# kchmck/p25rx

Hardware: AMD Instinct MI355X
Metric: IQ Msamples/s through FM-demod+C4FM slice (higher is better)
Workload: dtype f32

## Files before the change

### p25rx_amd/csrc/p25fe_api.hip

```cpp
#include "p25fe_kernels.hip"

#include <hip/hip_ext.h>
#include <math.h>
#include <stdio.h>
#include <stdlib.h>
#include <string.h>

#include <chrono>
#include <new>
#include <utility>
#include <string>
#include <vector>

#include "p25fe_jit.h"

using namespace p25k;

namespace {

constexpr size_t BBPAD = 256;
constexpr size_t SHARD_HALO = 2560;
static_assert(SHARD_HALO >= (size_t)(DEC * (PLPAD + CLK_L + 160) + TMAX) && 160 >= TMAX + TMAX - 1 && SHARD_HALO % 8 == 0, "shard halo");
constexpr uint32_t STATE_MAGIC = 0x50323546u;

// ... 685 lines not shown
}
struct K1Launch {
    const void* src = nullptr;
    int fmt = P25FE_FMT_CF32;
    size_t ch_stride = 0, n_hist = 0, n = 0;
    uint64_t abs0 = 0;
    float* bb = nullptr; size_t bb_stride = 0;
    float* power_dbm = nullptr;
    bool planar = false;
    K1Part part = K1_ALL;
    hipEvent_t ev0 = nullptr, ev1 = nullptr;
    const ChunkRecvArgs* chunk = nullptr;
    long* head_end = nullptr;
    unsigned* done_flag = nullptr; unsigned done_seq = 0u;
    hipStream_t stream = nullptr;
};

struct K1Plan {
    bool empty;
    K1Args a;
    int fmt, variant; bool ct; int pk;
    long n_seg;
    long head_end;
    size_t lds;
};
static int k1_plan(const p25fe_t* h, const K1Launch& L, K1Plan* p)
{
    const int fmt = L.fmt;
    const int variant = format_variant_of(h->variant, h->dflt, h->cfg.specialize, fmt);
    if (variant < 0) return variant;
    if ((reinterpret_cast<uintptr_t>(L.src) & 15u) != 0) return P25FE_ERR_ARG;
    if (h->C > 1 && (L.ch_stride % fmt_stride_unit(fmt)) != 0) return P25FE_ERR_ARG;
    if (L.chunk && (!L.planar || L.part)) return P25FE_ERR_ARG;
    const bool pro = seg_prologue(fmt);
    const long m_begin = !L.planar ? 0 : (pro ? -(long)PLPAD - h->look : -(long)HIST_BB - h->look);
    const size_t n_out = p25fe_n_baseband_h(h, L.abs0, L.n);
    const long total = (long)n_out - m_begin;
    K1Args& a = p->a;
    a.m_begin = m_begin; a.n_out = (long)n_out; p->head_end = 0;
    p->empty = total <= 0;
    if (p->empty) return P25FE_OK;
    const int pk = (L.planar || h->long_taps || variant == P25FE_VARIANT_SPECIALIZED) ? 5 : h->k1_p;
    const int t1 = h->long_taps ? TMAX : T1;
    static const long subs_env = [] { const char* e = getenv("P25FE_SUBS"); return e ? atol(e) : 0L; }();
    long subs = subs_env > 0 ? subs_env : (fmt == P25FE_FMT_U8 ? 9 : (fmt == P25FE_FMT_S16 ? P25FE_K1_SUBS_S16 : 3));
    if (L.chunk) subs = 1;
    if (subs > 32768) subs = 32768;
    const bool ct = variant != P25FE_VARIANT_GENERIC;
    const int t2e = h->long_taps ? TMAX : T2;
    const int t3geo = ct ? h->n_avg : TMAX;
    SegGeo g{pro, WV * pk, (int)subs, seg_halo_for(h->n_avg, t2e), 0, m_begin, (long)n_out};
    const int nd = g.front(t3geo, t2e);
    const long o0 = (long)(((uint64_t)h->phase + 5 - L.abs0 % 5) % 5);
    if (L.part && subs > 1 && !L.chunk) g.set_lead(nd, o0, t1);
    const long n_seg = g.count(total);
    const long pl_shift = PLPAD + h->look;
    if (L.planar && !g.planar_ok(pl_shift)) return P25FE_ERR_ARG;
    if (L.planar && n_out > MAX_RANGE_BB) return P25FE_ERR_ARG;
    long seg_first = 0, seg_count = n_seg;
    if (L.part) {
        if (L.power_dbm) return P25FE_ERR_ARG;
        const long k_min = g.head_count(n_seg, nd, o0, t1);
        if (L.part == K1_MAIN) { seg_first = k_min; seg_count = n_seg - k_min; }
        else seg_count = k_min;
        p->head_end = g.start(k_min) - m_begin;
        p->empty = seg_count <= 0;
        if (p->empty) return P25FE_OK;
    }
    if (seg_count * (long)h->C > 0x7fffffffL) return P25FE_ERR_ARG;
    p->fmt = fmt; p->variant = variant; p->ct = ct; p->pk = pk; p->n_seg = n_seg;
    a.x = L.src; a.ch_stride = (long)L.ch_stride; a.n_hist = (long)L.n_hist; a.n_new = (long)L.n; a.o0 = (int)o0; a.n_ch = h->C;
    a.bb = L.bb; a.bb_stride = (long)L.bb_stride; a.power_partial = nullptr;
    a.subs_per_seg = g.subs_per_seg; a.seg_first = (int)seg_first; a.seg_count = (int)seg_count; a.lead_segs = g.lead_segs; a.seg_halo = g.segh;
    a.bbp = nullptr; a.bbp_ch_stride = 0; a.bits = nullptr; a.bits_ch_stride = 0; a.pl_shift = (int)pl_shift;
    a.done_flag = L.planar ? L.done_flag : nullptr; a.done_seq = L.done_seq;
    if (L.planar) {
        const PlanarGeo g(n_out);
        a.bbp = h->rx().pl_f.get(); a.bbp_ch_stride = (long)g.floats();
        a.bits = reinterpret_cast<uint8_t*>(h->rx().pl_bits.get()); a.bits_ch_stride = (long)(4 * g.words());
    }
    const bool lut = fmt == P25FE_FMT_U8 && (!ct || h->u8_lut_mode);
    p->lds = h->long_taps ? k1_lds_bytes<Geo<5, 1>>(ct, lut, t3geo) : (pk == 3 ? k1_lds_bytes<Geo<3>>(ct, lut, t3geo) : k1_lds_bytes<Geo<5>>(ct, lut, t3geo));
    static const size_t lds_pad_env = [] { const char* e = getenv("P25FE_K1_LDS_PAD"); return e ? (size_t)atol(e) : (size_t)0; }();
    p->lds += lds_pad_env;
    return P25FE_OK;
}

using K1Kernel = void (*)(K1Args, const Taps*);
using ChunkKernel = void (*)(K1Args, const Taps*, ChunkTail);
template <int FMT> static K1Kernel k1_kernel_of(bool ct, int pk, bool planar, bool long_taps)
{
    if (long_taps) return planar ? k_frontend<FMT, false, 5, OUT_PLANAR, 1> : k_frontend<FMT, false, 5, OUT_LINEAR, 1>;
    if (planar) return ct ? k_frontend<FMT, true, 5, OUT_PLANAR, 0> : k_frontend<FMT, false, 5, OUT_PLANAR, 0>;
    if (pk == 3) return ct ? k_frontend<FMT, true, 3, OUT_LINEAR, 0> : k_frontend<FMT, false, 3, OUT_LINEAR, 0>;
    return ct ? k_frontend<FMT, true, 5, OUT_LINEAR, 0> : k_frontend<FMT, false, 5, OUT_LINEAR, 0>;
}
template <int FMT> static ChunkKernel chunk_kernel_of(bool ct, bool long_taps)
{
    if (long_taps) return k_chunk<FMT, false, 1>;
    return ct ? k_chunk<FMT, true, 0> : k_chunk<FMT, false, 0>;
}
static K1Kernel k1_kernel_of(int fmt, bool ct, int pk, bool planar, bool long_taps)
{
    switch (fmt) {
    case P25FE_FMT_U8: return k1_kernel_of<P25FE_FMT_U8>(ct, pk, planar, long_taps);
    case P25FE_FMT_S16: return k1_kernel_of<P25FE_FMT_S16>(ct, pk, planar, long_taps);
    default: return k1_kernel_of<P25FE_FMT_CF32>(ct, pk, planar, long_taps);
    }
}
static ChunkKernel chunk_kernel_of(int fmt, bool ct, bool long_taps)
{
    switch (fmt) {
    case P25FE_FMT_U8: return chunk_kernel_of<P25FE_FMT_U8>(ct, long_taps);
    case P25FE_FMT_S16: return chunk_kernel_of<P25FE_FMT_S16>(ct, long_taps);
    default: return chunk_kernel_of<P25FE_FMT_CF32>(ct, long_taps);
// ... 1427 lines not shown
```

### p25rx_amd/csrc/p25fe_jit.cpp

```cpp
#include "p25fe_jit.h"

#include <dlfcn.h>
#include <errno.h>
#include <fcntl.h>
#include <hip/hiprtc.h>
#include <math.h>
#include <stdio.h>
#include <stdlib.h>
#include <string.h>
#include <sys/stat.h>
#include <sys/types.h>
#include <unistd.h>

#include "p25fe_embed.inc"

namespace p25jit {

const char* const KERNEL_NAMES[2][3] = {
    {"p25jit_k1_cf32_lin", "p25jit_k1_cf32_pl", "p25jit_chunk_cf32"},
    {"p25jit_k1_u8_lin", "p25jit_k1_u8_pl", "p25jit_chunk_u8"},
};

static const char* const OPTIONS[] = {"--offload-arch=gfx950", "-O3", "-std=c++17", "-ffp-contract=off", "-fno-fast-math",
                                      "-fhip-fp32-correctly-rounded-divide-sqrt", "-Wno-unused-function"};
static const int N_OPTIONS = (int)(sizeof OPTIONS / sizeof OPTIONS[0]);

static const char WRAPPER[] =
    "#include \"p25fe_jit_spec.h\"\n"
    "#include \"p25fe_kernels.hip\"\n"
    "using namespace p25k;\n"
    "#define P25JIT_K1(NAME, FMT, OM, WPS) extern \"C\" __global__ __launch_bounds__(WV, WPS) void NAME(K1Args a, const Taps* __restrict__ t) "
    "{ frontend_body<FMT, true, 5, OM, P25FE_JIT_TX>(a, t); }\n"
    "P25JIT_K1(p25jit_k1_cf32_lin, P25FE_FMT_CF32, OUT_LINEAR, Geo<5>::WAVES_PER_SIMD)\n"
    "P25JIT_K1(p25jit_k1_u8_lin, P25FE_FMT_U8, OUT_LINEAR, Geo<5>::WAVES_PER_SIMD)\n"
    "P25JIT_K1(p25jit_k1_cf32_pl, P25FE_FMT_CF32, OUT_PLANAR, P25FE_K1_PLANAR_WPS)\n"
    "P25JIT_K1(p25jit_k1_u8_pl, P25FE_FMT_U8, OUT_PLANAR, (P25FE_JIT_AVG_N > AVG_DPP_MAX ? 2 : P25FE_K1_PLANAR_WPS_U8))\n"
    "extern \"C\" __global__ __launch_bounds__(WV, 2) void p25jit_chunk_cf32(K1Args a, const Taps* __restrict__ t, ChunkTail c) "
    "{ chunk_body<P25FE_FMT_CF32, true, P25FE_JIT_TX>(a, t, c); }\n"
    "extern \"C\" __global__ __launch_bounds__(WV, 2) void p25jit_chunk_u8(K1Args a, const Taps* __restrict__ t, ChunkTail c) "
    "{ chunk_body<P25FE_FMT_U8, true, P25FE_JIT_TX>(a, t, c); }\n";

namespace rtc {
struct Api {
    void* lib = nullptr;
    decltype(&hiprtcCreateProgram) create = nullptr;
    decltype(&hiprtcCompileProgram) compile = nullptr;
    decltype(&hiprtcGetProgramLogSize) log_size = nullptr;
    decltype(&hiprtcGetProgramLog) log = nullptr;
    decltype(&hiprtcGetCodeSize) code_size = nullptr;
    decltype(&hiprtcGetCode) code = nullptr;
    decltype(&hiprtcDestroyProgram) destroy = nullptr;
    decltype(&hiprtcGetErrorString) error_string = nullptr;
    decltype(&hiprtcVersion) version = nullptr;
    bool ok = false;
};
static const Api& api()
{
    static const Api a = [] {
        Api x;
        const char* env = getenv("P25FE_HIPRTC");
        const char* names[] = {"libhiprtc.so.7", "libhiprtc.so", "/opt/rocm/lib/libhiprtc.so"};
        if (env && *env) x.lib = dlopen(env, RTLD_NOW | RTLD_LOCAL);
        else
            for (const char* n : names)
                if ((x.lib = dlopen(n, RTLD_NOW | RTLD_LOCAL)) != nullptr) break;
        if (!x.lib) return x;
#define P25_SYM(field, name) x.field = reinterpret_cast<decltype(x.field)>(dlsym(x.lib, name))
        P25_SYM(create, "hiprtcCreateProgram"); P25_SYM(compile, "hiprtcCompileProgram");
// ... 262 lines not shown
```

### p25rx_amd/csrc/p25fe_kernels.hip

```cpp
#ifndef __HIPCC_RTC__
#include <hip/hip_runtime.h>
#include <stdint.h>
#endif

#include "p25fe.h"
#include "p25fe_spec.h"

namespace p25k {

#ifdef P25FE_MEASURE
#include "p25fe_measure.inc"
#else
#define P25FE_M_LOAD_OFFSET(product_, cached_row_) (product_)
#define P25FE_M_ENTRY do { } while (0)
#define P25FE_M_LOCALS do { } while (0)
#define P25FE_M_ITEM do { } while (0)
#define P25FE_M_SUBTILE do { } while (0)
#define P25FE_M_EXIT do { } while (0)
#define K1_STAMP(i) do { } while (0)
#define K1_PIN2(a, b) do { } while (0)
#define P25FE_M_PIN_V2(arr_, n_) do { } while (0)
#define P25FE_M_PIN_F2(arr_, n_) do { } while (0)
#define P25FE_M_CUT_LOADS do { } while (0)
#define P25FE_M_CUT(stage_) do { } while (0)
// ... 21 lines not shown
#define K1_CT_DECIM_TAPS P25FE_JIT_DECIM_TAPS
#define K1_CT_CHAN_TAPS P25FE_JIT_CHAN_TAPS
#define K1_CT_FM_GAIN P25FE_JIT_FM_GAIN
#define K1_CT_U8_SCALE P25FE_JIT_U8_SCALE
#define K1_CT_U8_OFFSET P25FE_JIT_U8_OFFSET
#define K1_CT_U8_LUT P25FE_JIT_U8_LUT
#define K1_CT_AVG_N P25FE_JIT_AVG_N
#define K1_CT_AVG_TAPS P25FE_JIT_AVG_TAPS
#define K1_CT_AVG_UNIFORM P25FE_JIT_AVG_UNIFORM
#else
#define K1_CT_DECIM_TAPS P25FE_DEFAULT_DECIM_TAPS
#define K1_CT_CHAN_TAPS P25FE_DEFAULT_CHAN_TAPS
#define K1_CT_FM_GAIN P25FE_FM_GAIN
#define K1_CT_U8_SCALE P25FE_U8_SCALE
#define K1_CT_U8_OFFSET P25FE_U8_OFFSET
#define K1_CT_U8_LUT 0
#define K1_CT_AVG_N P25FE_BOXCAR
#define K1_CT_AVG_TAPS P25FE_DEFAULT_AVG_TAPS
#define K1_CT_AVG_UNIFORM 1
#endif

constexpr int WV = 64;
constexpr int DEC = P25FE_DECIM;
constexpr int T1 = P25FE_T1;
constexpr int T2 = P25FE_T2;
constexpr int BOX = P25FE_BOXCAR;
constexpr int HALO_Y = BOX;
constexpr int HALO_D = HALO_Y + (T2 - 1);
constexpr int TMAX = P25FE_MAX_TAPS;
constexpr int AVG_DPP_MAX = 11;
constexpr int SEG_HALO = 80;
__host__ __device__ constexpr int seg_halo_for(int t3, int t2) { return t3 + t2 - 1 <= 80 ? 80 : 160; }
static_assert(SEG_HALO == seg_halo_for(BOX, TMAX) && seg_halo_for(TMAX, TMAX) >= TMAX + TMAX - 1, "segment halo covers the filter memory and is byte-aligned per plane");
#ifndef P25FE_K1_PRO_CF32
#define P25FE_K1_PRO_CF32 0
#endif
#ifndef P25FE_K1_PRO_S16
#define P25FE_K1_PRO_S16 1
#endif
__host__ __device__ constexpr bool seg_prologue(int fmt)
{
    return fmt == P25FE_FMT_U8 ? true : (fmt == P25FE_FMT_S16 ? P25FE_K1_PRO_S16 != 0 : P25FE_K1_PRO_CF32 != 0);
}
__host__ __device__ constexpr int fmt_bps(int fmt) { return fmt == P25FE_FMT_CF32 ? 8 : (fmt == P25FE_FMT_S16 ? 4 : 2); }

constexpr int SPS_ = P25FE_SPS;
constexpr int PLPAD = 320;
static_assert(PLPAD % 320 == 0 && PLPAD >= 240 + 2, "planar pad holds the receiver's history");
constexpr int OUT_LINEAR = 0, OUT_PLANAR = 1;
constexpr int PL_BLK = 32 * P25FE_SPS;
__host__ __device__ inline long planar_index(long i, int r) { return (i >> 5) * PL_BLK + r * 32 + (i & 31); }

#define K1_GEO_FN __host__ __device__ __forceinline__ constexpr
#define K1_FIRST_INPUT(m, o0, t1) ((long)(o0) + DEC * (m) - ((t1) - 1))
struct SegGeo {
    bool pro;
    int sub, subs_per_seg;
    int segh;
    int lead_segs;
    long m_begin, n_out;
    long seg_len_ = pro ? (long)subs_per_seg * sub : (long)(sub - segh) + (long)(subs_per_seg - 1) * sub;
    long lead_len_ = pro ? (long)sub : (long)(sub - segh);
    K1_GEO_FN long seg_len() const { return seg_len_; }
    K1_GEO_FN long lead_len() const { return lead_len_; }
    K1_GEO_FN SegGeo range(int lead, long mb, long no) const { SegGeo g = *this; g.lead_segs = lead; g.m_begin = mb; g.n_out = no; return g; }
    K1_GEO_FN bool is_lead(long k) const { return k < (long)lead_segs; }
    K1_GEO_FN long len(long k) const { return is_lead(k) ? lead_len_ : seg_len_; }
    K1_GEO_FN int subs(long k) const { return is_lead(k) ? 1 : subs_per_seg; }
    K1_GEO_FN long start(long k) const { return m_begin + (is_lead(k) ? k * lead_len_ : (long)lead_segs * lead_len_ + (k - lead_segs) * seg_len_); }
    K1_GEO_FN long end_of(long m0, long len_) const { return (m0 + len_ < n_out) ? m0 + len_ : n_out; }
    K1_GEO_FN long end(long k) const { return end_of(start(k), len(k)); }
    K1_GEO_FN long count(long total) const
    {
        return lead_segs * lead_len_ >= total ? (total + lead_len_ - 1) / lead_len_ : lead_segs + (total - lead_segs * lead_len_ + seg_len_ - 1) / seg_len_;
    }
    K1_GEO_FN int front(int t3geo, int t2) const { return pro ? t3geo + t2 - 1 : segh; }
    K1_GEO_FN static long first_input(long m, long o0, int t1) { return K1_FIRST_INPUT(m, o0, t1); }
    K1_GEO_FN bool in_head(long k, int front_, long o0, int t1) const { return first_input(start(k) - front_, o0, t1) < 0; }
    K1_GEO_FN long head_count(long n_seg, int front_, long o0, int t1) const { long k = 0; while (k < n_seg && in_head(k, front_, o0, t1)) ++k; return k; }
    K1_GEO_FN void set_lead(int front_, long o0, int t1) { for (lead_segs = 0; lead_segs < 64 && start(lead_segs) < n_out && in_head(lead_segs, front_, o0, t1);) ++lead_segs; }
    K1_GEO_FN bool planar_ok(long pl_shift) const
    {
// ... 3 lines not shown
};
#undef K1_GEO_FN
constexpr int HIST_IQ = DEC * HALO_D + (T1 - 1) + (DEC - 1);
constexpr int HIST_IQ_MAX = DEC * (TMAX + TMAX - 1) + (TMAX - 1) + (DEC - 1);

template <int PK, int TX = 0> struct Geo {
    static constexpr int T1 = TX ? TMAX : P25FE_T1;
    static constexpr int T2 = TX ? TMAX : P25FE_T2;
    static constexpr int D_CARRY = (T2 - 1 + 1) & ~1;
    static constexpr int P = PK;
    static constexpr int SUB = WV * PK;
    static constexpr int XWIN = DEC * SUB + (T1 - DEC);
    static constexpr int XIN_N = (XWIN + 1 + 7) / 8 * 8;
    static constexpr int D_N = D_CARRY + SUB;
    static constexpr int TAPS_N = T1 + T2 + 3 + TMAX + 1;
    static constexpr size_t LDS_BASE = sizeof(float2) * (D_CARRY + XIN_N);
    static_assert(sizeof(float2) * XIN_N >= sizeof(float2) * SUB + sizeof(float) * SUB, "d and the transpose fit the window region");
    static constexpr int WAVES_PER_SIMD = PK <= 3 ? 4 : 2;
};

struct Taps {
    float dec[TMAX];
    float ch[TMAX];
    float lut[256];
    float fm_gain;
    int n_avg;
    int avg_uniform;
    float pad_;
    float avg[TMAX];
};
#ifndef P25FE_K1_AVG_LDS_CF32
#define P25FE_K1_AVG_LDS_CF32 0
#endif
template <class G> __host__ __device__ constexpr size_t k1_lds_bytes(bool ct, bool lut, int t3)
{
    return G::LDS_BASE + sizeof(float) * (size_t)((ct ? 0 : G::TAPS_N) + (lut ? 256 : 0) + (t3 > AVG_DPP_MAX || !ct || P25FE_K1_AVG_LDS_CF32 ? t3 - 1 + G::SUB : 0));
}

__device__ __forceinline__ float spec_atan2f(float y, float x)
{
    const float ax = __builtin_fabsf(x), ay = __builtin_fabsf(y);
    const float mx = ax > ay ? ax : ay;
    const float mn = ax > ay ? ay : ax;
    const float t = mn / mx;
    const float s = t * t;
    float p = P25FE_ATAN_COEFFS[P25FE_ATAN_NCOEF - 1];
#pragma unroll
    for (int i = P25FE_ATAN_NCOEF - 2; i >= 0; --i) p = __builtin_fmaf(p, s, P25FE_ATAN_COEFFS[i]);
    float r = p * t;
    if (ay > ax) r = P25FE_HALF_PI - r;
    if (x < 0.0f) r = P25FE_PI - r;
    if (y < 0.0f) r = -r;
    return mx == 0.0f ? 0.0f : r;
}

__device__ __forceinline__ float fm_discriminate(float2 s, float2 prev, float gain)
{
    const float t = s.y * prev.y;
    const float re = __builtin_fmaf(s.x, prev.x, t);
    const float u = s.x * prev.y;
    const float im = __builtin_fmaf(s.y, prev.x, -u);
    return spec_atan2f(im, re) * gain;
}

typedef float v2f __attribute__((ext_vector_type(2)));
#ifndef P25FE_K1_SCALAR_FMA
#define P25FE_K1_SCALAR_FMA 0
#endif
__device__ __forceinline__ v2f cfma(float tap, v2f s, v2f acc)
// ... 147 lines not shown
        "v_writelane_b32 %0, %1, 0\n\tv_writelane_b32 %0, %2, 5\n\t"
        "v_writelane_b32 %0, %3, 1\n\tv_writelane_b32 %0, %4, 6\n\t"
        "v_writelane_b32 %0, %5, 2\n\tv_writelane_b32 %0, %6, 7\n\t"
        "v_writelane_b32 %0, %7, 3\n\tv_writelane_b32 %0, %8, 8\n\t"
        "v_writelane_b32 %0, %9, 4\n\tv_writelane_b32 %0, %10, 9"
        : "+v"(v)
        : "s"((unsigned)m[0]), "s"((unsigned)(m[0] >> 32)), "s"((unsigned)m[1]), "s"((unsigned)(m[1] >> 32)),
          "s"((unsigned)m[2]), "s"((unsigned)(m[2] >> 32)), "s"((unsigned)m[3]), "s"((unsigned)(m[3] >> 32)),
          "s"((unsigned)m[4]), "s"((unsigned)(m[4] >> 32)));
    return v;
}
__device__ __forceinline__ unsigned lane_gather(unsigned v, int src)
{
    return (unsigned)__builtin_amdgcn_ds_bpermute(src << 2, (int)v);
}

__device__ __forceinline__ void phase_sync()
{
    __builtin_amdgcn_fence(__ATOMIC_RELEASE, "wavefront");
    __builtin_amdgcn_wave_barrier();
    __builtin_amdgcn_fence(__ATOMIC_ACQUIRE, "wavefront");
}

__device__ __forceinline__ float u8_to_f32(unsigned b) { return __builtin_fmaf((float)b, K1_CT_U8_SCALE, K1_CT_U8_OFFSET); }
__device__ __forceinline__ float2 s16_to_c32(unsigned w)
{
    const int i = (int)(short)(w & 0xffffu), q = (int)w >> 16;
    return make_float2((float)i * P25FE_S16_SCALE, (float)q * P25FE_S16_SCALE);
}

#ifndef P25FE_K1_LD_AUX
#define P25FE_K1_LD_AUX 0
#endif
template <int FMT, int PK, int TX = 0, int NVX = 0> struct Loader {
    using G = Geo<PK, TX>;
    static constexpr int LOG_SPV = 1;
    static constexpr int SPV = 1 << LOG_SPV;
    static constexpr int NV = NVX ? NVX : (G::XWIN + SPV + SPV * WV - 1) / (SPV * WV);
    static_assert(FMT == P25FE_FMT_CF32 || FMT == P25FE_FMT_S16 || FMT == P25FE_FMT_U8, "input format");
    using V = typename cond<FMT == P25FE_FMT_CF32, uint4, typename cond<FMT == P25FE_FMT_S16, uint2, unsigned>::type>::type;
    V v[NV];

    typedef unsigned v4u_t __attribute__((ext_vector_type(4)));
    typedef unsigned v2u_t __attribute__((ext_vector_type(2)));
    static constexpr int BPS = fmt_bps(FMT);
    static constexpr int VB = BPS * SPV;
    __device__ __forceinline__ void load_vec(int j, int o)
    {
        if constexpr (FMT == P25FE_FMT_CF32) {
            const v4u_t t = __builtin_amdgcn_raw_buffer_load_b128(rs, o, 0, P25FE_K1_LD_AUX);
            v[j] = make_uint4(t.x, t.y, t.z, t.w);
        } else if constexpr (FMT == P25FE_FMT_S16) {
            const v2u_t t = __builtin_amdgcn_raw_buffer_load_b64(rs, o, 0, P25FE_K1_LD_AUX);
            v[j] = make_uint2(t.x, t.y);
        } else {
            v[j] = __builtin_amdgcn_raw_buffer_load_b32(rs, o, 0, P25FE_K1_LD_AUX);
        }
    }
    __amdgpu_buffer_rsrc_t rs;
    long base_idx;

    __device__ __forceinline__ void init(const void* base, long first0, long n_hist, long n_new, long i_last)
    {
        const long f_al = (first0 >> LOG_SPV) << LOG_SPV;
        const long lo_al = ((-n_hist) >> LOG_SPV) << LOG_SPV;
        base_idx = f_al > lo_al ? f_al : lo_al;
        const long last = i_last < n_new - 1 ? i_last : n_new - 1;
        long bytes = ((last + 1 - base_idx + SPV - 1) >> LOG_SPV) * VB;
        bytes = bytes < 0 ? 0 : (bytes > (1L << 30) ? (1L << 30) : bytes);
        const uintptr_t p = reinterpret_cast<uintptr_t>(base) + (uintptr_t)(base_idx * BPS);
        const unsigned plo = __builtin_amdgcn_readfirstlane((unsigned)p), phi = __builtin_amdgcn_readfirstlane((unsigned)(p >> 32));
        rs = __builtin_amdgcn_make_buffer_rsrc(reinterpret_cast<void*>(((uintptr_t)phi << 32) | plo), 0,
                                               __builtin_amdgcn_readfirstlane((int)bytes), 0x00020000);
    }
    __device__ __forceinline__ void load_first(long first, int tid)
    {
        const long f_al = (first >> LOG_SPV) << LOG_SPV;
        long rel = (f_al - base_idx) * BPS;
        rel = rel < -(1L << 30) ? -(1L << 30) : (rel > (1L << 30) ? (1L << 30) : rel);
        const int voff = (int)rel + VB * tid;
#pragma unroll
        for (int j = 0; j < NV; ++j) {
            int o = voff + j * VB * WV;
            o = o < 0 ? 0x7ffffff0 : o;
            load_vec(j, o);
        }
    }
    __device__ __forceinline__ void load(long first, int tid)
    {
        const long f_al = (first >> LOG_SPV) << LOG_SPV;
        long rel = (f_al - base_idx) * BPS;
        rel = rel < -(1L << 30) ? -(1L << 30) : (rel > (1L << 30) ? (1L << 30) : rel);
        const int voff = (int)rel + VB * tid;
#pragma unroll
        for (int j = 0; j < NV; ++j) {
            const int o = P25FE_M_LOAD_OFFSET(voff + j * VB * WV, VB * tid);
            load_vec(j, o);
        }
    }

    template <bool LUTM = false>
    __device__ __forceinline__ void store(float2* XIN, long first, long n_hist, long n_new, int tid, const float* lut = nullptr) const
    {
        float4* XV = reinterpret_cast<float4*>(__builtin_assume_aligned(XIN, 16));
#pragma unroll
        for (int j = 0; j < NV; ++j) {
            float2 s[SPV];
#pragma unroll
            for (int e = 0; e < SPV; ++e) {
                if constexpr (FMT == P25FE_FMT_CF32) {
                    const unsigned w[4] = {v[j].x, v[j].y, v[j].z, v[j].w};
                    s[e] = make_float2(__uint_as_float(w[2 * e]), __uint_as_float(w[2 * e + 1]));
                } else if constexpr (FMT == P25FE_FMT_S16) {
                    s[e] = s16_to_c32(e ? v[j].y : v[j].x);
                } else {
                    const unsigned pair = (v[j] >> (16 * e)) & 0xffffu;
                    if constexpr (LUTM) s[e] = make_float2(lut[pair & 0xffu], lut[pair >> 8]);
                    else s[e] = make_float2(u8_to_f32(pair & 0xffu), u8_to_f32(pair >> 8));
                }
            }
            if (j < NV - 1 || SPV * (tid + j * WV) + SPV <= G::XIN_N) XV[tid + j * WV] = make_float4(s[0].x, s[0].y, s[1].x, s[1].y);
        }
    }
    __device__ __forceinline__ void fixup(float2* XIN, long first, long n_hist, long n_new, int tid) const
    {
        const long first_al = (first >> LOG_SPV) << LOG_SPV;
        if (first_al >= -n_hist && first_al + (long)NV * SPV * WV <= n_new) return;
#pragma unroll
        for (int j = 0; j < NV; ++j)
#pragma unroll
            for (int e = 0; e < SPV; ++e) {
                const long i = first_al + SPV * (long)(tid + j * WV) + e;
                const int k = SPV * (tid + j * WV) + e;
                if ((i < -n_hist || i >= n_new) && k < G::XIN_N) XIN[k] = make_float2(0.f, 0.f);
            }
    }
};

struct K1Args {
    const void* x;
    long ch_stride;
    long n_hist;
    long n_new;
    int o0;
    float* bb;
    long bb_stride;
    long n_out;
    int subs_per_seg;
    int seg_count;
    int n_ch;
    int seg_first;
    long m_begin;
    float* power_partial;
    float* bbp;
    long bbp_ch_stride;
    uint8_t* bits;
    long bits_ch_stride;
    int pl_shift;
    unsigned* done_flag;
    unsigned done_seq;
    int lead_segs;
    int seg_halo;
};

#ifndef P25FE_K1_PLANAR_WPS
#define P25FE_K1_PLANAR_WPS 2
#endif
#ifndef P25FE_K1_PLANAR_WPS_U8
#define P25FE_K1_PLANAR_WPS_U8 3
#endif
#ifndef P25FE_K1_PLANAR_WPS_S16
#define P25FE_K1_PLANAR_WPS_S16 3
#endif
#ifndef P25FE_K1_TURNAROUND_PRIO
#define P25FE_K1_TURNAROUND_PRIO 3
#endif
#ifndef P25FE_K1_PF_CF32
#define P25FE_K1_PF_CF32 1
#endif
#ifndef P25FE_K1_NT_STORES
#define P25FE_K1_NT_STORES 1
#endif
#ifndef P25FE_K1_PF_U8
#define P25FE_K1_PF_U8 2
#endif
#ifndef P25FE_K1_SUBS_S16
#define P25FE_K1_SUBS_S16 9
#endif
#ifndef P25FE_K1_PF_S16
#define P25FE_K1_PF_S16 1
#endif
template <int FMT, bool CT, int PK, int OM = OUT_LINEAR, int TX = 0>
__device__ __forceinline__ void frontend_body(const K1Args& a, const Taps* __restrict__ gtaps)
{
    constexpr int PF = (PK != 5 || TX != 0) ? 1 : (FMT == P25FE_FMT_U8 ? P25FE_K1_PF_U8 : (FMT == P25FE_FMT_S16 ? P25FE_K1_PF_S16 : P25FE_K1_PF_CF32));
#ifndef P25FE_JIT
    static_assert(TX == 0 || !CT, "the 64-tap geometry is for caller-supplied taps");
#endif
    static_assert(OM == OUT_LINEAR || PK == 5, "the planar epilogue maps a 320-sample sub-tile onto 10 planes x 32 symbols");
    P25FE_M_ENTRY;
    using G = Geo<PK, TX>;
    constexpr int SUB = G::SUB;
    constexpr int P = PK;
    constexpr int T1 = G::T1, T2 = G::T2, D_CARRY = G::D_CARRY;
    constexpr int T3 = CT ? K1_CT_AVG_N : TMAX;
    constexpr bool AVG_DPP = CT && T3 <= AVG_DPP_MAX && !(P25FE_K1_AVG_LDS_CF32 != 0 && FMT == P25FE_FMT_CF32);
    constexpr int HY = T3;
    constexpr int NBACK = AVG_DPP ? ((T3 - 1 + PK - 1) / PK > 0 ? (T3 - 1 + PK - 1) / PK : 1) : 1;
    static_assert(T3 >= 1 && T3 <= TMAX && NBACK <= 3, "post-discriminator filter length");
    extern __shared__ __attribute__((aligned(16))) char smem[];
    float2* D = reinterpret_cast<float2*>(smem);
    float2* XIN = D + D_CARRY;
    float* OUT = reinterpret_cast<float*>(D + G::D_N);
    float* TAPS = reinterpret_cast<float*>(D + D_CARRY + G::XIN_N);
    float* const LUT = TAPS + (CT ? 0 : G::TAPS_N);
    float* const AVT = TAPS + (T1 + T2 + 3);
    constexpr bool LUTM = FMT == P25FE_FMT_U8 && (!CT || K1_CT_U8_LUT != 0);
    const int tid = threadIdx.x;
    if (!CT) {
        for (int k = tid; k < T1; k += WV) TAPS[k] = gtaps->dec[k];
        for (int k = tid; k < T2; k += WV) TAPS[T1 + k] = gtaps->ch[k];
        for (int k = tid; k < TMAX; k += WV) AVT[k] = gtaps->avg[k];
    }
    if constexpr (LUTM)
        for (int k = tid; k < 256; k += WV) LUT[k] = gtaps->lut[k];
    float* const FM = LUT + (LUTM ? 256 : 0);
    float fm_gain = K1_CT_FM_GAIN;
    int n_avg = T3, avg_uniform = K1_CT_AVG_UNIFORM;
    if constexpr (!CT) {
        fm_gain = __int_as_float(__builtin_amdgcn_readfirstlane(__float_as_int(gtaps->fm_gain)));
        n_avg = __builtin_amdgcn_readfirstlane(gtaps->n_avg);
        avg_uniform = __builtin_amdgcn_readfirstlane(gtaps->avg_uniform);
    }
    const int SEGH = CT ? seg_halo_for(T3, T2) : a.seg_halo;
    auto tap_dec = [&](int k) -> float { return CT ? K1_CT_DECIM_TAPS[k] : TAPS[k]; };
    auto tap_ch = [&](int k) -> float { return CT ? K1_CT_CHAN_TAPS[k] : TAPS[T1 + k]; };

    constexpr bool PRO = seg_prologue(FMT);
    const SegGeo shape{PRO, SUB, a.subs_per_seg, SEGH};
    constexpr int ND = SegGeo{true}.front(HY, T2);
    constexpr int PWIN = DEC * (ND - 1) + T1;
    constexpr int NVP = (PWIN + 2 + 2 * WV - 1) / (2 * WV);
    constexpr int PBASE = 2 * WV * NVP;
    constexpr int NDL = (ND + WV - 1) / WV;
    static_assert(PBASE + ND <= G::XIN_N && D_CARRY <= ND, "prologue scratch fits the window region");
    P25FE_M_LOCALS;
    const long n_items = (long)a.seg_count * a.n_ch;
    const bool grid2d = gridDim.x == (unsigned)a.seg_count;
    for (long item = grid2d ? (long)blockIdx.y * a.seg_count + blockIdx.x : (long)blockIdx.x; item < n_items;
         item += grid2d ? n_items : (long)gridDim.x) {
    P25FE_M_ITEM;
    const int ch = grid2d ? (int)blockIdx.y : (int)((unsigned)item / (unsigned)a.seg_count);
    const long seg_rel = grid2d ? (long)blockIdx.x : item - (long)ch * a.seg_count;
    const long seg = seg_rel + a.seg_first;
    const SegGeo sg = shape.range(a.lead_segs, a.m_begin, a.n_out);
    const long this_len = sg.len(seg);
    const int subs_this = sg.subs(seg);
    const long m_seg0 = sg.start(seg);
    if (m_seg0 >= a.n_out) continue;
    const long m_seg1 = sg.end_of(m_seg0, this_len);
    const char* xb = reinterpret_cast<const char*>(a.x) + (size_t)ch * a.ch_stride * fmt_bps(FMT);
    float* bb = a.bb + (size_t)ch * a.bb_stride;
    phase_sync();

    using LoaderT = Loader<FMT, PK, TX>;
    using LoaderP = Loader<FMT, PK, TX, NVP>;
    LoaderT ld0, ld1;
    long dlo = PRO ? m_seg0 : m_seg0 - sg.front(HY, T2);
    const long i_last = (long)a.o0 + DEC * (m_seg1 - 1);
    float pw = 0.f;
    float2 y_carry = make_float2(0.f, 0.f);
    float f_carry[NBACK][P];
    if constexpr (!PRO) {
        for (int k = tid; k < D_CARRY; k += WV) D[k] = make_float2(0.f, 0.f);
        if constexpr (!AVG_DPP)
            for (int k = tid; k < T3 - 1; k += WV) FM[k] = 0.f;
        ld0.init(xb, K1_FIRST_INPUT(dlo, a.o0, T1), a.n_hist, a.n_new, i_last);
        ld0.load_first(K1_FIRST_INPUT(dlo, a.o0, T1), tid);
        if constexpr (PF == 2) {
            ld1.rs = ld0.rs; ld1.base_idx = ld0.base_idx;
            ld1.load(K1_FIRST_INPUT(dlo + SUB, a.o0, T1), tid);
        }
#pragma unroll
        for (int b = 0; b < NBACK; ++b)
#pragma unroll
            for (int p = 0; p < P; ++p) f_carry[b][p] = 0.f;
    } else {
    LoaderP lp;
    const long pfirst = K1_FIRST_INPUT(m_seg0 - ND, a.o0, T1);
    ld0.init(xb, pfirst, a.n_hist, a.n_new, i_last);
    lp.rs = ld0.rs; lp.base_idx = ld0.base_idx;
    lp.load_first(pfirst, tid);
    constexpr bool LATE_LD0 = FMT == P25FE_FMT_CF32;
    if constexpr (!LATE_LD0) {
        ld0.load_first(K1_FIRST_INPUT(dlo, a.o0, T1), tid);
        if constexpr (PF == 2) {
            ld1.rs = ld0.rs; ld1.base_idx = ld0.base_idx;
            ld1.load_first(K1_FIRST_INPUT(dlo + SUB, a.o0, T1), tid);
        }
    }
    {
        float2* const PD_ = XIN + PBASE;
        lp.template store<LUTM>(XIN, pfirst, a.n_hist, a.n_new, tid, LUT);
        lp.fixup(XIN, pfirst, a.n_hist, a.n_new, tid);
        if constexpr (LATE_LD0) {
            ld0.load_first(K1_FIRST_INPUT(dlo, a.o0, T1), tid);
            if constexpr (PF == 2) {
                ld1.rs = ld0.rs; ld1.base_idx = ld0.base_idx;
                ld1.load_first(K1_FIRST_INPUT(dlo + SUB, a.o0, T1), tid);
            }
        }
        phase_sync();
        const int pxsh = (int)(pfirst & 1);
        v2f dacc[NDL];
#pragma unroll
        for (int r = 0; r < NDL; ++r) {
            dacc[r] = v2f{0.f, 0.f};
            const int l = tid + WV * r;
            if (NDL == 1 || l < ND) {
                const float2* w = XIN + pxsh + DEC * l;
                lds_walk<T1, CT>(w, [&](auto jc, v2f sv) {
                    constexpr int j = decltype(jc)::value;
                    dacc[r] = cfma(tap_dec(T1 - 1 - j), sv, dacc[r]);
                });
            }
        }
#pragma unroll
        for (int r = 0; r < NDL; ++r) {
            const int l = tid + WV * r;
            if (l < ND) PD_[l] = make_float2(dacc[r].x, dacc[r].y);
        }
        phase_sync();
        v2f yv = v2f{0.f, 0.f};
        if (tid < HY) {
            const float2* w = PD_ + (ND - HY) - (T2 - 1) + tid;
            lds_walk<T2, CT>(w, [&](auto jc, v2f sv) {
                constexpr int j = decltype(jc)::value;
                yv = cfma(tap_ch(T2 - 1 - j), sv, yv);
            });
        }
        float2 yp;
        yp.x = wave_shr1(yv.x, 0.f);
        yp.y = wave_shr1(yv.y, 0.f);
        const float fmv = fm_discriminate(make_float2(yv.x, yv.y), yp, fm_gain);
        y_carry.x = lane_bcast<HY - 1>(yv.x);
        y_carry.y = lane_bcast<HY - 1>(yv.y);
        static_for<0, NBACK>([&](auto bc) {
            constexpr int b = decltype(bc)::value;
            static_for<0, P>([&](auto pc) {
                constexpr int p = decltype(pc)::value;
                constexpr int l = HY - (b + 1) * P + p;
                if constexpr (AVG_DPP && l >= 1) f_carry[b][p] = lane_bcast<l>(fmv);
                else f_carry[b][p] = 0.f;
            });
        });
        if constexpr (!AVG_DPP)
            if (tid >= 1 && tid < HY) FM[tid - 1] = fmv;
        for (int k = tid; k < D_CARRY; k += WV) D[k] = PD_[ND - D_CARRY + k];
        phase_sync();
    }
    }

    float outv[P];
// ... 251 lines not shown
        } else {
            unsigned w = 0u;
            unsigned long long sg[5];
#pragma unroll
            for (int q = 0; q < P; ++q) {
                outv[q] = OUT[SPS_ * pl_sym + pl_h5 + q];
                sg[q] = __builtin_amdgcn_ballot_w64(__float_as_int(outv[q]) < 0);
            }
            if constexpr (!P25FE_M_NO_SIGN_PLANES) w = lanes_from_ballots(sg);
            if constexpr (PRO) {
                bitsv = w;
            } else {
                const unsigned pw_ = lane_gather(w, tid >> 2);
                bitsv = (pw_ >> (8 * (tid & 3))) & 0xffu;
            }
        }
        out_rel = (int)(dlo - m_seg0);
        phase_sync();
        K1_PIN2(outv[0], outv[P - 1]);
        K1_STAMP(6);
        return true;
    };
    if constexpr (PF == 1) {
        for (int it = 0; it < subs_this; ++it, dlo += SUB)
            if (!sub_tile(ld0)) break;
    } else {
        for (int it = 0; it < subs_this; it += 2) {
            if (!sub_tile(ld0)) break;
            dlo += SUB;
            if (it + 1 >= subs_this || !sub_tile(ld1)) break;
            dlo += SUB;
        }
    }
    flush_outputs();

    if (a.power_partial) {
#pragma unroll
        for (int d = 32; d > 0; d >>= 1) pw = pw + __shfl_down(pw, d, 64);
        if (tid == 0) a.power_partial[(size_t)ch * a.seg_count + seg_rel] = pw;
    }
    }
    if constexpr (OM == OUT_PLANAR) {
        if (a.done_flag) {
            asm volatile("s_waitcnt vmcnt(0)" ::: "memory");
            __builtin_amdgcn_fence(__ATOMIC_RELEASE, "agent");
            asm volatile("s_waitcnt vmcnt(0)" ::: "memory");
            unsigned ticket = 0u;
            if (tid == 0) ticket = __hip_atomic_fetch_add(a.done_flag + 1, 1u, __ATOMIC_RELAXED, __HIP_MEMORY_SCOPE_AGENT);
            ticket = (unsigned)__builtin_amdgcn_readfirstlane((int)ticket);
            if (ticket == gridDim.x * gridDim.y - 1u) {
                __builtin_amdgcn_fence(__ATOMIC_ACQUIRE, "agent");
                if (tid == 0) {
                    __hip_atomic_store(a.done_flag + 1, 0u, __ATOMIC_RELAXED, __HIP_MEMORY_SCOPE_AGENT);
                    __hip_atomic_store(a.done_flag, a.done_seq, __ATOMIC_RELEASE, __HIP_MEMORY_SCOPE_AGENT);
                }
            }
        }
    }
    P25FE_M_EXIT;
}

constexpr int k1_wps(int fmt, bool ct, int pk, int om)
{
    if (om == OUT_PLANAR)
        return fmt == P25FE_FMT_U8 ? (ct ? P25FE_K1_PLANAR_WPS_U8 : 2) : (fmt == P25FE_FMT_S16 ? (ct ? P25FE_K1_PLANAR_WPS_S16 : 2) : P25FE_K1_PLANAR_WPS);
    return (fmt == P25FE_FMT_U8 && !ct && pk <= 3) ? 3 : (pk <= 3 ? 4 : 2);
}
template <int FMT, bool CT, int PK, int OM = OUT_LINEAR, int TX = 0>
__global__ __launch_bounds__(WV, k1_wps(FMT, CT, PK, OM)) void k_frontend(K1Args a, const Taps* __restrict__ gtaps)
{
    frontend_body<FMT, CT, PK, OM, TX>(a, gtaps);
}

constexpr int PD = P25FE_PRE_DECIM;
constexpr int T0 = P25FE_T0;
#ifndef P25FE_K0_P
#define P25FE_K0_P 3
#endif
constexpr int K0_P = P25FE_K0_P;
constexpr int K0_SUB = WV * K0_P;
#ifndef P25FE_K0_SUBS
#define P25FE_K0_SUBS 2
#endif
#ifndef P25FE_K0_WPS
#define P25FE_K0_WPS 2
#endif
constexpr int K0_SUBS = P25FE_K0_SUBS;
constexpr int K0_HALO = T0 - PD;
constexpr int K0_NIN = PD * K0_SUB + K0_HALO;
constexpr int k0_row_pitch(int need) { return need + ((13 - need % 16) + 16) % 16; }
constexpr int K0_JP = k0_row_pitch(K0_NIN / PD + 2);
static_assert(K0_JP >= K0_NIN / PD + 2 && K0_JP % 16 == 13, "polyphase row pitch");
constexpr int K0_NV = (K0_NIN + 2 + 2 * WV - 1) / (2 * WV);
constexpr int HIST_PRE = K0_HALO + PD - 1;

struct K0Args {
    const float* x;
    long ch_stride;
    long n_hist, n_new;
    int o0;
    float* y;
    long y_stride;
// ... 694 lines not shown
    unsigned long long acc[3] = {words, errs, fixed};
#pragma unroll
    for (int q = 0; q < 3; ++q) {
#pragma unroll
        for (int o = 32; o > 0; o >>= 1) acc[q] += __shfl_down(acc[q], o, 64);
        if ((tid & 63) == 0) sh[q][tid >> 6] = acc[q];
    }
    __syncthreads();
    if (tid == 0) {
        p25fe_chan_stats_t o;
        o.sig_power_dbm = power_dbm ? power_dbm[ch] : __int_as_float(0x7fc00000);
        o.locked = r.anchor_out.valid != 0 ? 1 : 0;
        o.n_dibits = r.n_dibits;
        o.n_sync = r.n_sync;
        o.last_sync_pos = (r.n_sync > 0 && r.anchor_out.valid) ? r.anchor_out.s : -1;
        o.bch.words = sh[0][0] + sh[0][1] + sh[0][2] + sh[0][3];
        o.bch.errs = sh[1][0] + sh[1][1] + sh[1][2] + sh[1][3];
        o.bch.fixed = sh[2][0] + sh[2][1] + sh[2][2] + sh[2][3];
        o.bch.size = 63; o.bch.reserved = 0;
        stats[ch] = o;
    }
}
#endif

struct ChunkTail {
    ChunkRecvArgs r;
    unsigned* counter;
    int wg_per_ch;
};

template <int FMT, bool CT, int TX>
__device__ __forceinline__ void chunk_body(const K1Args& a, const Taps* __restrict__ gtaps, const ChunkTail& t)
{
    frontend_body<FMT, CT, 5, OUT_PLANAR, TX>(a, gtaps);
    asm volatile("s_waitcnt vmcnt(0)" ::: "memory");
    __builtin_amdgcn_fence(__ATOMIC_RELEASE, "agent");
    asm volatile("s_waitcnt vmcnt(0)" ::: "memory");
    unsigned ticket = 0u;
    if (threadIdx.x == 0) ticket = __hip_atomic_fetch_add(&t.counter[blockIdx.y], 1u, __ATOMIC_RELAXED, __HIP_MEMORY_SCOPE_AGENT);
    ticket = (unsigned)__builtin_amdgcn_readfirstlane((int)ticket);
    if (ticket != (unsigned)t.wg_per_ch - 1u) return;
    __builtin_amdgcn_fence(__ATOMIC_ACQUIRE, "agent");
    if (threadIdx.x == 0) t.counter[blockIdx.y] = 0u;
    recv_one_tile(t.r, (int)blockIdx.y);
}

template <int FMT, bool CT, int TX>
__global__ __launch_bounds__(WV, 2) void k_chunk(K1Args a, const Taps* __restrict__ gtaps, ChunkTail t)
{
    chunk_body<FMT, CT, TX>(a, gtaps, t);
}


#ifndef P25FE_JIT
__global__ __launch_bounds__(256) void k_shard_compact(const uint8_t* gathered, unsigned long long cap, const uint64_t* offset,
                                                        int first_shard, int n_shards, uint8_t* out, unsigned long long out_cap)
{
    const int r = first_shard + (int)blockIdx.y;
    if (r >= n_shards) return;
    const unsigned long long o0 = offset[r], n = offset[r + 1] - o0;
    const uint8_t* src = gathered + (unsigned long long)r * cap;
    for (unsigned long long i = (unsigned long long)blockIdx.x * 256 + threadIdx.x; i < n && i < cap; i += (unsigned long long)gridDim.x * 256)
        if (o0 + i < out_cap) out[o0 + i] = src[i];
}
#endif

#ifndef P25FE_JIT
// ... 29 lines not shown
```

Before: 523,400.

## Load part of cf32 planar window via buffer-to-LDS DMA with prologue and higher occupancy

```diff
diff --git a/p25rx_amd/csrc/p25fe_api.hip b/p25rx_amd/csrc/p25fe_api.hip
--- a/p25rx_amd/csrc/p25fe_api.hip
+++ b/p25rx_amd/csrc/p25fe_api.hip
@@ -741,7 +741,8 @@
     if ((reinterpret_cast<uintptr_t>(L.src) & 15u) != 0) return P25FE_ERR_ARG;
     if (h->C > 1 && (L.ch_stride % fmt_stride_unit(fmt)) != 0) return P25FE_ERR_ARG;
     if (L.chunk && (!L.planar || L.part)) return P25FE_ERR_ARG;
-    const bool pro = seg_prologue(fmt);
+    const bool hyb = k1_cf32_product(fmt, variant != P25FE_VARIANT_GENERIC, 5, L.planar ? OUT_PLANAR : OUT_LINEAR, h->long_taps ? 1 : 0, h->n_avg, L.chunk != nullptr);
+    const bool pro = seg_prologue(fmt, hyb);
     const long m_begin = !L.planar ? 0 : (pro ? -(long)PLPAD - h->look : -(long)HIST_BB - h->look);
     const size_t n_out = p25fe_n_baseband_h(h, L.abs0, L.n);
     const long total = (long)n_out - m_begin;
@@ -789,7 +790,7 @@
         a.bits = reinterpret_cast<uint8_t*>(h->rx().pl_bits.get()); a.bits_ch_stride = (long)(4 * g.words());
     }
     const bool lut = fmt == P25FE_FMT_U8 && (!ct || h->u8_lut_mode);
-    p->lds = h->long_taps ? k1_lds_bytes<Geo<5, 1>>(ct, lut, t3geo) : (pk == 3 ? k1_lds_bytes<Geo<3>>(ct, lut, t3geo) : k1_lds_bytes<Geo<5>>(ct, lut, t3geo));
+    p->lds = h->long_taps ? k1_lds_bytes<Geo<5, 1>>(ct, lut, t3geo) : (pk == 3 ? k1_lds_bytes<Geo<3>>(ct, lut, t3geo) : k1_lds_bytes<Geo<5>>(ct, lut, t3geo, hyb));
     static const size_t lds_pad_env = [] { const char* e = getenv("P25FE_K1_LDS_PAD"); return e ? (size_t)atol(e) : (size_t)0; }();
     p->lds += lds_pad_env;
     return P25FE_OK;
diff --git a/p25rx_amd/csrc/p25fe_jit.cpp b/p25rx_amd/csrc/p25fe_jit.cpp
--- a/p25rx_amd/csrc/p25fe_jit.cpp
+++ b/p25rx_amd/csrc/p25fe_jit.cpp
@@ -33,7 +33,7 @@
     "{ frontend_body<FMT, true, 5, OM, P25FE_JIT_TX>(a, t); }\n"
     "P25JIT_K1(p25jit_k1_cf32_lin, P25FE_FMT_CF32, OUT_LINEAR, Geo<5>::WAVES_PER_SIMD)\n"
     "P25JIT_K1(p25jit_k1_u8_lin, P25FE_FMT_U8, OUT_LINEAR, Geo<5>::WAVES_PER_SIMD)\n"
-    "P25JIT_K1(p25jit_k1_cf32_pl, P25FE_FMT_CF32, OUT_PLANAR, P25FE_K1_PLANAR_WPS)\n"
+    "P25JIT_K1(p25jit_k1_cf32_pl, P25FE_FMT_CF32, OUT_PLANAR, k1_wps(P25FE_FMT_CF32, true, 5, OUT_PLANAR, P25FE_JIT_TX))\n"
     "P25JIT_K1(p25jit_k1_u8_pl, P25FE_FMT_U8, OUT_PLANAR, (P25FE_JIT_AVG_N > AVG_DPP_MAX ? 2 : P25FE_K1_PLANAR_WPS_U8))\n"
     "extern \"C\" __global__ __launch_bounds__(WV, 2) void p25jit_chunk_cf32(K1Args a, const Taps* __restrict__ t, ChunkTail c) "
     "{ chunk_body<P25FE_FMT_CF32, true, P25FE_JIT_TX>(a, t, c); }\n"
diff --git a/p25rx_amd/csrc/p25fe_kernels.hip b/p25rx_amd/csrc/p25fe_kernels.hip
--- a/p25rx_amd/csrc/p25fe_kernels.hip
+++ b/p25rx_amd/csrc/p25fe_kernels.hip
@@ -77,15 +77,12 @@
 constexpr int SEG_HALO = 80;
 __host__ __device__ constexpr int seg_halo_for(int t3, int t2) { return t3 + t2 - 1 <= 80 ? 80 : 160; }
 static_assert(SEG_HALO == seg_halo_for(BOX, TMAX) && seg_halo_for(TMAX, TMAX) >= TMAX + TMAX - 1, "segment halo covers the filter memory and is byte-aligned per plane");
-#ifndef P25FE_K1_PRO_CF32
-#define P25FE_K1_PRO_CF32 0
-#endif
 #ifndef P25FE_K1_PRO_S16
 #define P25FE_K1_PRO_S16 1
 #endif
-__host__ __device__ constexpr bool seg_prologue(int fmt)
-{
-    return fmt == P25FE_FMT_U8 ? true : (fmt == P25FE_FMT_S16 ? P25FE_K1_PRO_S16 != 0 : P25FE_K1_PRO_CF32 != 0);
+__host__ __device__ constexpr bool seg_prologue(int fmt, bool product = false)
+{
+    return fmt == P25FE_FMT_U8 ? true : (fmt == P25FE_FMT_S16 ? P25FE_K1_PRO_S16 != 0 : product);
 }
 __host__ __device__ constexpr int fmt_bps(int fmt) { return fmt == P25FE_FMT_CF32 ? 8 : (fmt == P25FE_FMT_S16 ? 4 : 2); }
 
@@ -93,6 +90,11 @@
 constexpr int PLPAD = 320;
 static_assert(PLPAD % 320 == 0 && PLPAD >= 240 + 2, "planar pad holds the receiver's history");
 constexpr int OUT_LINEAR = 0, OUT_PLANAR = 1;
+__host__ __device__ constexpr bool k1_cf32_product(int fmt, bool ct, int pk, int om, int tx, int t3, bool chunk)
+{
+    return fmt == P25FE_FMT_CF32 && ct && pk == 5 && om == OUT_PLANAR && tx == 0 && t3 <= AVG_DPP_MAX && !chunk;
+}
+constexpr int K1_LAND_BYTES = 2 * 16 * 64;
 constexpr int PL_BLK = 32 * P25FE_SPS;
 __host__ __device__ inline long planar_index(long i, int r) { return (i >> 5) * PL_BLK + r * 32 + (i & 31); }
 
@@ -162,9 +164,10 @@
 #ifndef P25FE_K1_AVG_LDS_CF32
 #define P25FE_K1_AVG_LDS_CF32 0
 #endif
-template <class G> __host__ __device__ constexpr size_t k1_lds_bytes(bool ct, bool lut, int t3)
-{
-    return G::LDS_BASE + sizeof(float) * (size_t)((ct ? 0 : G::TAPS_N) + (lut ? 256 : 0) + (t3 > AVG_DPP_MAX || !ct || P25FE_K1_AVG_LDS_CF32 ? t3 - 1 + G::SUB : 0));
+template <class G> __host__ __device__ constexpr size_t k1_lds_bytes(bool ct, bool lut, int t3, bool land = false)
+{
+    return G::LDS_BASE + sizeof(float) * (size_t)((ct ? 0 : G::TAPS_N) + (lut ? 256 : 0) + (t3 > AVG_DPP_MAX || !ct || P25FE_K1_AVG_LDS_CF32 ? t3 - 1 + G::SUB : 0)) +
+           (land ? K1_LAND_BYTES : 0);
 }
 
 __device__ __forceinline__ float spec_atan2f(float y, float x)
@@ -378,14 +381,21 @@
 #ifndef P25FE_K1_LD_AUX
 #define P25FE_K1_LD_AUX 0
 #endif
-template <int FMT, int PK, int TX = 0, int NVX = 0> struct Loader {
+template <int FMT, int PK, int TX = 0, int NVX = 0, int NDMA = 0> struct Loader {
     using G = Geo<PK, TX>;
     static constexpr int LOG_SPV = 1;
     static constexpr int SPV = 1 << LOG_SPV;
+    static constexpr int VBYTES_DMA = 16;
     static constexpr int NV = NVX ? NVX : (G::XWIN + SPV + SPV * WV - 1) / (SPV * WV);
     static_assert(FMT == P25FE_FMT_CF32 || FMT == P25FE_FMT_S16 || FMT == P25FE_FMT_U8, "input format");
     using V = typename cond<FMT == P25FE_FMT_CF32, uint4, typename cond<FMT == P25FE_FMT_S16, uint2, unsigned>::type>::type;
     V v[NV];
+    static constexpr int JD0 = NV - 1 - NDMA;
+    static_assert(NDMA == 0 || (FMT == P25FE_FMT_CF32 && NDMA * VBYTES_DMA * WV <= K1_LAND_BYTES && JD0 > 0 && SPV * WV * (JD0 + NDMA) <= G::XIN_N),
+                  "the DMA vectors are whole vectors of the window's interior and fit the landing area");
+    static constexpr bool is_dma(int j) { return NDMA > 0 && j >= JD0 && j < JD0 + NDMA; }
+    unsigned land;
+    int rec_bytes;
 
     typedef unsigned v4u_t __attribute__((ext_vector_type(4)));
     typedef unsigned v2u_t __attribute__((ext_vector_type(2)));
@@ -403,6 +413,12 @@
             v[j] = __builtin_amdgcn_raw_buffer_load_b32(rs, o, 0, P25FE_K1_LD_AUX);
         }
     }
+    __device__ __forceinline__ void dma_vec(int jd, int o) const
+    {
+        unsigned keep;
+        asm volatile("s_nop 4\n\ts_mov_b32 %0, m0\n\ts_mov_b32 m0, %3\n\ts_nop 0\n\tbuffer_load_dwordx4 %1, %2, 0 offen lds\n\ts_mov_b32 m0, %0"
+                     : "=&s"(keep) : "v"(o), "s"(rs), "s"(land + (unsigned)(jd * VBYTES_DMA * WV)) : "memory");
+    }
     __amdgpu_buffer_rsrc_t rs;
     long base_idx;
 
@@ -416,8 +432,8 @@
         bytes = bytes < 0 ? 0 : (bytes > (1L << 30) ? (1L << 30) : bytes);
         const uintptr_t p = reinterpret_cast<uintptr_t>(base) + (uintptr_t)(base_idx * BPS);
         const unsigned plo = __builtin_amdgcn_readfirstlane((unsigned)p), phi = __builtin_amdgcn_readfirstlane((unsigned)(p >> 32));
-        rs = __builtin_amdgcn_make_buffer_rsrc(reinterpret_cast<void*>(((uintptr_t)phi << 32) | plo), 0,
-                                               __builtin_amdgcn_readfirstlane((int)bytes), 0x00020000);
+        rec_bytes = __builtin_amdgcn_readfirstlane((int)bytes);
+        rs = __builtin_amdgcn_make_buffer_rsrc(reinterpret_cast<void*>(((uintptr_t)phi << 32) | plo), 0, rec_bytes, 0x00020000);
     }
     __device__ __forceinline__ void load_first(long first, int tid)
     {
@@ -429,7 +445,8 @@
         for (int j = 0; j < NV; ++j) {
             int o = voff + j * VB * WV;
             o = o < 0 ? 0x7ffffff0 : o;
-            load_vec(j, o);
+            if (is_dma(j)) dma_vec(j - JD0, o);
+            else load_vec(j, o);
         }
     }
     __device__ __forceinline__ void load(long first, int tid)
@@ -439,9 +456,12 @@
         rel = rel < -(1L << 30) ? -(1L << 30) : (rel > (1L << 30) ? (1L << 30) : rel);
         const int voff = (int)rel + VB * tid;
 #pragma unroll
+        for (int j = 0; j < NV; ++j)
+            if (is_dma(j)) dma_vec(j - JD0, P25FE_M_LOAD_OFFSET(voff + j * VB * WV, VB * tid));
+#pragma unroll
         for (int j = 0; j < NV; ++j) {
             const int o = P25FE_M_LOAD_OFFSET(voff + j * VB * WV, VB * tid);
-            load_vec(j, o);
+            if (!is_dma(j)) load_vec(j, o);
         }
     }
 
@@ -451,6 +471,7 @@
         float4* XV = reinterpret_cast<float4*>(__builtin_assume_aligned(XIN, 16));
 #pragma unroll
         for (int j = 0; j < NV; ++j) {
+            if (is_dma(j)) continue;
             float2 s[SPV];
 #pragma unroll
             for (int e = 0; e < SPV; ++e) {
@@ -467,11 +488,36 @@
             }
             if (j < NV - 1 || SPV * (tid + j * WV) + SPV <= G::XIN_N) XV[tid + j * WV] = make_float4(s[0].x, s[0].y, s[1].x, s[1].y);
         }
+        if constexpr (NDMA > 0) {
+            asm volatile("s_waitcnt vmcnt(0)" ::: "memory");
+            phase_sync();
+            const float4* LV = reinterpret_cast<const float4*>(__builtin_assume_aligned(reinterpret_cast<const char*>(XIN) + land_offset, 16));
+#pragma unroll
+            for (int jd = 0; jd < NDMA; ++jd) XV[tid + (JD0 + jd) * WV] = LV[tid + jd * WV];
+            dma_fixup(XIN, first, tid);
+        }
+    }
+    int land_offset;
+    __device__ __forceinline__ void dma_fixup(float2* XIN, long first, int tid) const
+    {
+        const long f_al = (first >> LOG_SPV) << LOG_SPV;
+        long rel = (f_al - base_idx) * BPS;
+        rel = rel < -(1L << 30) ? -(1L << 30) : (rel > (1L << 30) ? (1L << 30) : rel);
+        const int r0 = (int)rel + JD0 * VB * WV;
+        if (r0 >= 0 && r0 + NDMA * VB * WV <= rec_bytes) return;
+        asm volatile("" : "+v"(tid));
+        float4* XV = reinterpret_cast<float4*>(__builtin_assume_aligned(XIN, 16));
+#pragma unroll
+        for (int jd = 0; jd < NDMA; ++jd) {
+            const int o = r0 + VB * tid + jd * VB * WV;
+            if (o < 0 || o >= rec_bytes) XV[tid + (JD0 + jd) * WV] = make_float4(0.f, 0.f, 0.f, 0.f);
+        }
     }
     __device__ __forceinline__ void fixup(float2* XIN, long first, long n_hist, long n_new, int tid) const
     {
         const long first_al = (first >> LOG_SPV) << LOG_SPV;
         if (first_al >= -n_hist && first_al + (long)NV * SPV * WV <= n_new) return;
+        if constexpr (NDMA > 0) asm volatile("" : "+v"(tid));
 #pragma unroll
         for (int j = 0; j < NV; ++j)
 #pragma unroll
@@ -536,7 +582,7 @@
 #ifndef P25FE_K1_PF_S16
 #define P25FE_K1_PF_S16 1
 #endif
-template <int FMT, bool CT, int PK, int OM = OUT_LINEAR, int TX = 0>
+template <int FMT, bool CT, int PK, int OM = OUT_LINEAR, int TX = 0, bool CHUNK = false>
 __device__ __forceinline__ void frontend_body(const K1Args& a, const Taps* __restrict__ gtaps)
 {
     constexpr int PF = (PK != 5 || TX != 0) ? 1 : (FMT == P25FE_FMT_U8 ? P25FE_K1_PF_U8 : (FMT == P25FE_FMT_S16 ? P25FE_K1_PF_S16 : P25FE_K1_PF_CF32));
@@ -582,14 +628,16 @@
     auto tap_dec = [&](int k) -> float { return CT ? K1_CT_DECIM_TAPS[k] : TAPS[k]; };
     auto tap_ch = [&](int k) -> float { return CT ? K1_CT_CHAN_TAPS[k] : TAPS[T1 + k]; };
 
-    constexpr bool PRO = seg_prologue(FMT);
+    constexpr bool HYB = k1_cf32_product(FMT, CT, PK, OM, TX, T3, CHUNK);
+    constexpr bool PRO = seg_prologue(FMT, HYB);
+    static_assert(!HYB || (AVG_DPP && !LUTM), "the landing area sits where the window region ends: no taps, table or fm window behind it");
     const SegGeo shape{PRO, SUB, a.subs_per_seg, SEGH};
     constexpr int ND = SegGeo{true}.front(HY, T2);
     constexpr int PWIN = DEC * (ND - 1) + T1;
     constexpr int NVP = (PWIN + 2 + 2 * WV - 1) / (2 * WV);
     constexpr int PBASE = 2 * WV * NVP;
     constexpr int NDL = (ND + WV - 1) / WV;
-    static_assert(PBASE + ND <= G::XIN_N && D_CARRY <= ND, "prologue scratch fits the window region");
+    static_assert(PBASE + ND <= G::XIN_N && PBASE + WV * NDL <= G::XIN_N && D_CARRY <= ND, "prologue scratch fits the window region");
     P25FE_M_LOCALS;
     const long n_items = (long)a.seg_count * a.n_ch;
     const bool grid2d = gridDim.x == (unsigned)a.seg_count;
@@ -609,9 +657,13 @@
     float* bb = a.bb + (size_t)ch * a.bb_stride;
     phase_sync();
 
-    using LoaderT = Loader<FMT, PK, TX>;
+    using LoaderT = Loader<FMT, PK, TX, 0, HYB ? 2 : 0>;
     using LoaderP = Loader<FMT, PK, TX, NVP>;
     LoaderT ld0, ld1;
+    if constexpr (HYB) {
+        ld0.land_offset = (int)(sizeof(float2) * G::XIN_N);
+        ld0.land = (unsigned)(uintptr_t)(__attribute__((address_space(3))) char*)smem + (unsigned)G::LDS_BASE;
+    }
     long dlo = PRO ? m_seg0 : m_seg0 - sg.front(HY, T2);
     const long i_last = (long)a.o0 + DEC * (m_seg1 - 1);
     float pw = 0.f;
@@ -674,7 +726,7 @@
 #pragma unroll
         for (int r = 0; r < NDL; ++r) {
             const int l = tid + WV * r;
-            if (l < ND) PD_[l] = make_float2(dacc[r].x, dacc[r].y);
+            if (l < ND || (HYB && NDL == 1)) PD_[l] = make_float2(dacc[r].x, dacc[r].y);
         }
         phase_sync();
         v2f yv = v2f{0.f, 0.f};
@@ -992,6 +1044,7 @@
             dlo += SUB;
         }
     }
+    if constexpr (HYB) asm volatile("s_waitcnt vmcnt(0)" ::: "memory");
     flush_outputs();
 
     if (a.power_partial) {
@@ -1020,14 +1073,15 @@
     P25FE_M_EXIT;
 }
 
-constexpr int k1_wps(int fmt, bool ct, int pk, int om)
-{
+constexpr int k1_wps(int fmt, bool ct, int pk, int om, int tx = 0)
+{
+    if (k1_cf32_product(fmt, ct, pk, om, tx, K1_CT_AVG_N, false)) return 3;
     if (om == OUT_PLANAR)
         return fmt == P25FE_FMT_U8 ? (ct ? P25FE_K1_PLANAR_WPS_U8 : 2) : (fmt == P25FE_FMT_S16 ? (ct ? P25FE_K1_PLANAR_WPS_S16 : 2) : P25FE_K1_PLANAR_WPS);
     return (fmt == P25FE_FMT_U8 && !ct && pk <= 3) ? 3 : (pk <= 3 ? 4 : 2);
 }
 template <int FMT, bool CT, int PK, int OM = OUT_LINEAR, int TX = 0>
-__global__ __launch_bounds__(WV, k1_wps(FMT, CT, PK, OM)) void k_frontend(K1Args a, const Taps* __restrict__ gtaps)
+__global__ __launch_bounds__(WV, k1_wps(FMT, CT, PK, OM, TX)) void k_frontend(K1Args a, const Taps* __restrict__ gtaps)
 {
     frontend_body<FMT, CT, PK, OM, TX>(a, gtaps);
 }
@@ -1788,7 +1842,7 @@
 template <int FMT, bool CT, int TX>
 __device__ __forceinline__ void chunk_body(const K1Args& a, const Taps* __restrict__ gtaps, const ChunkTail& t)
 {
-    frontend_body<FMT, CT, 5, OUT_PLANAR, TX>(a, gtaps);
+    frontend_body<FMT, CT, 5, OUT_PLANAR, TX, true>(a, gtaps);
     asm volatile("s_waitcnt vmcnt(0)" ::: "memory");
     __builtin_amdgcn_fence(__ATOMIC_RELEASE, "agent");
     asm volatile("s_waitcnt vmcnt(0)" ::: "memory");
```

Result: slower. 514,200 (-1.8%).
